# yhw-yhw/TalkSHOW

Hardware: AMD Instinct MI355X
Metric: generated SMPL-X frames/sec (10 s @ 30 fps clips), whole job (higher is better)
Workload: dtype f32; 1 GPU; BASELINE configs[1]: batch=32 x 10 s clips, body+hand VQ-VAE encode -> PixelCNN greedy decode -> VQ decode, 30 fps; batch_per_gpu=32, frames_per_clip=300, coalesce=8, streams=3

## Files before the change

include/talkshow_hip_debug.h:

```cpp
#ifndef TALKSHOW_HIP_DEBUG_H
#define TALKSHOW_HIP_DEBUG_H

#include "talkshow_hip.h"

#ifdef __cplusplus
extern "C" {
#endif

int ts_stream_create_cus(ts_ctx *ctx, int cu_first, int cu_count, void **out_stream);
int ts_debug_skinny_trace(unsigned long long *out, int max_records);
int ts_debug_clock_sample(unsigned long long *dev_out, int n, int window_us, void *stream);
int ts_debug_conv_bands(int M, int N, int groups, int *out4);
int ts_debug_split_tile(int bid, int MT, int NT, int gw, int *out2);
int ts_debug_tile_weights(const float *W, int N, int K, long ldw, int epi, int gateD, float *out);

int ts_op_conv1d_timed(ts_ctx *ctx, const float *x_dev, int B, int Lin, int Cin, const float *w_packed_dev,
                       const float *bias_dev, int Cout, int K, int tile, int iters, float *out_dev, float *ms_out,
                       void *stream);
int ts_op_conv1d_strided_timed(ts_ctx *ctx, const float *x_dev, int B, int Lin, int Cin, const float *w_packed_dev,
                               const float *bias_dev, int Cout, int K, int stride, int tile, int iters, float *out_dev,
                               float *ms_out, void *stream);

int ts_op_conv_taps48_timed(ts_ctx *ctx, const float *x_dev, int B, int T, int G, int ntap, const float *w_dev, const float *bias_dev,
                            const float *res_dev, int iters, float *out_dev, float *ms_out, void *stream);
// ... 102 lines not shown
int ts_debug_mfcc_mel(ts_mfcc *m, const float *power, const int32_t *frames_dev, int B, int T, float *mel, void *stream);
int ts_debug_mfcc_db(ts_mfcc *m, float *mel, const int32_t *frames_dev, int B, int T, void *stream);
int ts_debug_mfcc_dct(ts_mfcc *m, const float *mel, const int32_t *frames_dev, int B, int T, float *feat, void *stream);

int ts_debug_smplx_dims(const ts_smplx *m, int32_t *out5);
int ts_debug_smplx_need(const ts_smplx *m, int32_t *verts_out);
int ts_debug_smplx_pose_prepare(ts_smplx *m, const float *betas, int betas_per_row, const float *rows, int row_ld, int expr_off, int64_t N,
                                float *rot_out, float *X_out, void *stream);
int ts_debug_smplx_blend(ts_smplx *m, int which, const float *X, int64_t N, float *out, void *stream);
int ts_debug_smplx_rigid_chain(ts_smplx *m, const float *rot, const float *jrest, int64_t N, float *G_out, float *A_out, float *joints_out,
                               void *stream);
int ts_debug_smplx_skin(ts_smplx *m, int full, const float *vposed, const float *A, int64_t N, float *out, void *stream);
int ts_debug_smplx_joints_tail(ts_smplx *m, const float *vs, int64_t N, float *joints, void *stream);

int ts_debug_pixelcnn_graphs(ts_pixelcnn *pix, void *stream);

int ts_debug_code_tables_plan(int V, int D, int B, int r, int j, int last_row, const char *knob_list, int64_t *out12);
int ts_debug_pixelcnn_tables(ts_pixelcnn *pix, int mode);
int64_t ts_debug_pixelcnn_work(ts_pixelcnn *pix, void *stream, int which, float *buf_dev, int64_t cap_floats, int put);
int ts_debug_code_table_stage(ts_pixelcnn *pix, int which, const int32_t *tok_dev, int B, const float *add1, const float *add2, const float *cls,
                              float *pre, float *out, float *q1, float *q0, void *stream);

int ts_debug_mixed_plan(const int32_t *hrows, int B, int max_counts, int32_t *active_out);

int ts_debug_rep_table(const ts_repeat *rep_host, int n_rep, int B, int V, int32_t *words_out);

int ts_op_vq_argmin_pair_masked(ts_ctx *ctx, const float *z_body_dev, const float *z_hand_dev, const int32_t *lens_dev, int B, int H_max,
                                const float *codebook_body_dev, const float *codebook_hand_dev, int ncode_body, int ncode_hand, int dim_body,
                                int dim_hand, int64_t *codes_dev, void *stream);
int ts_debug_vq_argmin_pair_masked(ts_ctx *ctx, const float *z_body_dev, const float *z_hand_dev, const int32_t *lens_dev, int B, int H_max,
                                   const float *codebook_body_dev, const float *codebook_hand_dev, int ncode_body, int ncode_hand,
                                   int dim_body, int dim_hand, int64_t *codes_dev, int form, int iters, void *stream);

int ts_debug_skinny_chain(ts_ctx *ctx, int M, int K, int gate, int iters, int debug, float *us_out);

#ifdef __cplusplus
}
#endif
#endif
```

talkshow_amd/_lib.py:

```python
import ctypes as C
import os

import numpy as np
import torch

_HERE = os.path.dirname(os.path.abspath(__file__))
LIB_PATH = os.environ.get("TS_LIB_PATH") or os.path.join(_HERE, "lib", "libtalkshow_hip.so")

TS_SAMPLE_GREEDY, TS_SAMPLE_UNIFORMS, TS_SAMPLE_PHILOX, TS_TEACHER_FORCED = 0, 1, 2, 3


class TsTensor(C.Structure):
    _fields_ = [("name", C.c_char_p), ("data", C.POINTER(C.c_float)), ("ndim", C.c_int32), ("shape", C.c_int64 * 4)]


_vp, _i, _i64, _u64, _fp = C.c_void_p, C.c_int, C.c_int64, C.c_uint64, C.POINTER(C.c_float)


class TsSampling(C.Structure):
    _fields_ = [("temperature", C.c_float), ("top_p", C.c_float), ("top_k", C.c_int32), ("reserved", C.c_int32)]


_sp = C.POINTER(TsSampling)

# ... 113 lines not shown
    "ts_resample_kaiser": (_i, [_vp, _vp, _i, C.c_long, _i, _i, _vp, _vp]),
    "ts_mfcc_forward_mixed": (_i, [_vp, _vp, C.POINTER(C.c_int32), _vp, _i, C.c_long, _vp, _vp]),
    "ts_mfcc_resample_mixed": (_i, [_vp, _vp, C.POINTER(C.c_int32), _vp, _i, C.c_long, _vp, _vp]),
    "ts_resample_kaiser_mixed": (_i, [_vp, _vp, C.POINTER(C.c_int32), _vp, _i, C.c_long, _i, _i, _vp, _vp]),
    "ts_debug_mfcc_stft": (_i, [_vp, _vp, _i, C.c_long, _vp, _vp]),
    "ts_debug_mfcc_stft_lens": (_i, [_vp, _vp, C.POINTER(C.c_int32), _vp, _i, C.c_long, _vp, _vp]),
    "ts_debug_mfcc_frames": (_i, [_vp, _vp, _i, C.c_long, _vp, _vp]),
    "ts_debug_mfcc_mel": (_i, [_vp, _vp, _vp, _i, _i, _vp, _vp]),
    "ts_debug_mfcc_db": (_i, [_vp, _vp, _vp, _i, _i, _vp]),
    "ts_debug_mfcc_dct": (_i, [_vp, _vp, _vp, _i, _i, _vp, _vp]),
    "ts_pixelcnn_graph_stats": (_i, [_vp, _vp, _i, _i, _i, C.POINTER(_i64), C.POINTER(C.c_double)]),
    "ts_body_pixel_infer": (_i, [_vp, _vp, _vp, _vp, _vp, _vp, _i, _i, _i, _vp, _u64, _i64, _vp, _vp, _vp]),
    "ts_body_pixel_infer_mixed": (_i, [_vp, _vp, _vp, _vp, _vp, _vp, C.POINTER(C.c_int32), _vp, _i, _i, _i, _vp, _u64, _vp, _vp, _vp, _vp]),
    "ts_audioenc_forward_masked": (_i, [_vp, _vp, _vp, _i, _i, _vp, _vp]),
    "ts_pixelcnn_generate_mixed": (_i, [_vp, _vp, _vp, C.POINTER(C.c_int32), _vp, _i, _i, _i, _vp, _u64, _vp, _vp, _vp]),
    "ts_vqvae_decode_pair_masked": (_i, [_vp, _vp, _vp, _vp, _vp, _i, _i, _vp, _vp]),
    "ts_debug_mixed_plan": (_i, [C.POINTER(C.c_int32), _i, _i, C.POINTER(C.c_int32)]),
    "ts_body_vq_infer": (_i, [_vp, _vp, _vp, _i, _i, _vp, _vp, _vp]),
    "ts_op_conv1d": (_i, [_vp, _vp, _i, _i, _i, _fp, _fp, _i, _i, _i, _i, _i, _i, _vp, _vp]),
    "ts_op_conv1d_timed": (_i, [_vp, _vp, _i, _i, _i, _vp, _vp, _i, _i, _i, _i, _vp, C.POINTER(C.c_float), _vp]),
    "ts_op_conv_taps48_timed": (_i, [_vp, _vp, _i, _i, _i, _i, _vp, _vp, _vp, _i, _vp, C.POINTER(C.c_float), _vp]),
    "ts_op_conv1d_strided_timed": (_i, [_vp, _vp, _i, _i, _i, _vp, _vp, _i, _i, _i, _i, _i, _vp, C.POINTER(C.c_float), _vp]),
    "ts_debug_pixelcnn_graphs": (_i, [_vp, _vp]),
    "ts_debug_code_tables_plan": (_i, [_i, _i, _i, _i, _i, _i, C.c_char_p, C.POINTER(_i64)]),
    "ts_debug_pixelcnn_tables": (_i, [_vp, _i]),
    "ts_debug_pixelcnn_work": (_i64, [_vp, _vp, _i, _vp, _i64, _i]),
    "ts_debug_code_table_stage": (_i, [_vp, _i, _vp, _i, _vp, _vp, _vp, _vp, _vp, _vp, _vp, _vp]),
    "ts_debug_conv_run": (_i, [_vp, C.POINTER(ConvProblem), _i, C.c_char_p, _i, C.POINTER(_i), _vp]),
    "ts_debug_conv_sk_plan": (_i, [_i, _i, _i, _i, C.POINTER(C.c_int)]),
    "ts_debug_conv_sk_run": (_i, [_i, _i, _i, _i, C.POINTER(C.c_int)]),
    "ts_debug_conv_sk_supported": (_i, []),
    "ts_pixelcnn_graph_captures": (C.c_long, [_vp, _vp]),
    "ts_pixelcnn_prepare": (_i, [_vp, _i, _i, _i, _vp]),
    "ts_debug_conv_plan": (_i, [_i, _i, _i, _i, _i, C.POINTER(_i), _i, _i, C.c_char_p, C.POINTER(_i)]),
    "ts_debug_skinny_plan": (_i, [C.POINTER(_i), _i, C.c_char_p, C.POINTER(_i)]),
    "ts_debug_skinny_run": (_i, [_vp, C.POINTER(SkinnyProblem), _i, C.c_char_p, C.POINTER(_i), _vp]),
    "ts_debug_gate_act": (_i, [_vp, _vp, _vp, C.c_long, _vp]),
    "ts_debug_gelu": (_i, [_vp, _vp, C.c_long, _vp]),
    "ts_debug_attention": (_i, [_vp, _i, _i, _i, _i, C.c_float, _vp, _vp]),
    "ts_debug_layernorm_rows": (_i, [_vp, _i, C.c_long, _i, _vp, _vp, _vp, _i, _i, _vp, _i, _vp]),
    "ts_debug_lerp_ln": (_i, [_vp, _i, _i, _i, _vp, _vp, _vp, _vp]),
    "ts_debug_w2v_conv0": (_i, [_vp, _i, _i, _vp, _vp, _vp, _i, _vp, _vp]),
    "ts_debug_fill_id": (_i, [_vp, _i, _vp, _vp, _i, _vp, _i, _i, _i, _i, _vp]),
    "ts_debug_attention_mixed": (_i, [_vp, C.POINTER(C.c_int32), _vp, _i, _i, _i, _i, C.c_float, _vp, _vp]),
    "ts_debug_layernorm_rows_lens": (_i, [_vp, _i, _i, _i, _vp, _i, _vp, _vp, _vp, _i, _i, _vp, _i, _vp]),
    "ts_debug_lerp_ln_lens": (_i, [_vp, _i, _i, _i, _vp, _vp, _vp, _vp, _vp, _vp]),
    "ts_debug_w2v_conv0_lens": (_i, [_vp, _i, _i, _vp, _vp, _vp, _vp, _i, _vp, _vp]),
    "ts_debug_fill_id_lens": (_i, [_vp, _i, _vp, _vp, _i, _vp, _i, _i, _i, _i, _vp, _vp]),
    "ts_debug_face_mixed_grid": (_i, [C.POINTER(C.c_int32), _i, _i, C.POINTER(C.c_int32), _i]),
    "ts_debug_face_packed_layout": (_i, [C.POINTER(C.c_int32), C.POINTER(C.c_int32), _i, C.POINTER(_i64), C.POINTER(_i64), C.POINTER(_i64)]),
    "ts_debug_face_generate_mixed": (_i, [_vp, _vp, C.POINTER(C.c_int32), _vp, C.POINTER(C.c_int32), _vp, _i, _i, _i, _vp, _vp, _vp, _vp, _i]),
    "ts_debug_attention_packed": (_i, [_vp, C.POINTER(C.c_int32), _vp, _i, _i, _i, C.c_float, _vp, _vp]),
    "ts_debug_pack_rows": (_i, [_vp, C.POINTER(C.c_int32), _i, _i, _i, _vp, _vp]),
    "ts_debug_unpack_rows": (_i, [_vp, C.POINTER(C.c_int32), _vp, _i, _i, _i, _vp, _vp]),
    "ts_debug_w2v_conv0_packed": (_i, [_vp, _i, _i, C.POINTER(C.c_int32), _vp, _vp, _vp, _vp, _i, _vp, _vp]),
    "ts_debug_lerp_ln_packed": (_i, [_vp, _i, _i, C.POINTER(C.c_int32), _vp, _vp, _vp, _vp, _vp, _vp]),
    "ts_op_vq_argmin": (_i, [_vp, _vp, _i, _vp, _i, _i, _vp, _vp]),
    "ts_op_linear": (_i, [_vp, _vp, _i, _i, _fp, _fp, _i, _i, _vp, _vp]),
    "ts_op_sample": (_i, [_vp, _vp, _i, _i, _i, _vp, _vp, _vp]),
    "ts_op_sample_philox": (_i, [_vp, _vp, _i, _i, _u64, _i64, C.c_uint32, _vp, _vp]),
    "ts_debug_skinny_chain": (_i, [_vp, _i, _i, _i, _i, _i, C.POINTER(C.c_float)]),
    "ts_smplx_create": (_i, [_vp, _i, _i, _i, _i, _fp, _fp, _fp, _fp, C.POINTER(C.c_int32), _fp, _fp, C.POINTER(C.c_int32), _i,
                             C.POINTER(C.c_int32), _i, C.POINTER(C.c_int32), _fp, _i, C.POINTER(_vp)]),
    "ts_smplx_destroy": (None, [_vp]),
    "ts_smplx_num_joints": (_i, [_vp]),
    "ts_smplx_forward": (_i, [_vp, _vp, _i, _vp, _i, _i, _i64, _vp, _vp, _vp]),
# ... 595 lines not shown
```

talkshow_amd/csrc/api.cpp:

```cpp
#include <cstring>
#include <vector>
#include "host_common.h"
#include "conv_tile.h"
#include "skinny_desc.h"

using namespace ts;

namespace {
struct BodyWork {
    DevBuf feat;
    DevBuf lat[2];
    DevBuf given;
};
BodyWork &body_work(hipStream_t s) {
    static StreamWorks<BodyWork> works;
    return works.get(s);
}
}

namespace ts {
template <class Get>
static Knobs read_knobs(Get get) {
    Knobs v;
    auto num = [&](const char *name, int dflt) { const char *e = get(name); return e && e[0] ? std::atoi(e) : dflt; };
    v.conv_bands = num("TS_CONV_BANDS", 1) != 0;
    v.conv_ring = num("TS_CONV_RING", 9);
    v.conv_deal = num("TS_CONV_DEAL", 1) != 0;
    v.conv_ring_paired = num("TS_CONV_RING_PAIRED", 1) != 0;
    v.conv_taps48 = num("TS_CONV_TAPS48", 1) != 0;
    v.face_pack = num("TS_FACE_PACK", 0) != 0;
    v.conv_sk = num("TS_CONV_SK", 1);
    v.w2v_moments = num("TS_W2V_MOMENTS", 1) != 0;
    v.vq_lds = num("TS_VQ_LDS", 1) != 0;
    v.vq_pair = num("TS_VQ_PAIR", 1) != 0;
    v.split_xcd = num("TS_SPLIT_XCD", 8);
    v.prof_log = num("TS_PROF_LOG", 0) != 0;
    if (const char *e = get("TS_NO_GRAPH")) v.no_graph = e[0] && e[0] != '0';
    v.pix_defer_p = num("TS_PIX_DEFER_P", -1);
    v.pix_tables = num("TS_PIX_TABLES", -1);
    v.skinny_v = num("TS_SKINNY_V", 1);
    v.skinny_nt = num("TS_SKINNY_NT", 16);
    v.skinny_tiled = num("TS_SKINNY_TILED", 1) != 0;
    v.wide_min = num("TS_SKINNY_WIDE_MIN", 160);
    v.skinny_shape = num("TS_SKINNY_SHAPE", 0);
    v.skinny_trace = num("TS_SKINNY_TRACE", 0);
    v.wide_ablate = num("TS_SKINNY_WIDE_ABLATE", 0);
    v.wide_pair = num("TS_SKINNY_WIDE_PAIR", 1) != 0;
    return v;
}
const Knobs &knobs() {
    static const Knobs k = read_knobs([](const char *name) { return std::getenv(name); });
    return k;
}
static Knobs knobs_from_list(const char *list) {
    return read_knobs([list](const char *name) -> const char * {
        const size_t n = std::strlen(name);
        for (const char *q = list; q && (q = std::strstr(q, name)); q += n)
            if ((q == list || q[-1] == ',' || q[-1] == ' ') && q[n] == '=') return q + n + 1;
        return nullptr;
    });
}
}

extern "C" {
// ... 1114 lines not shown
    sp.tok32 = tok.i();
    sp.tok_stride = 1;
    sp.codes = idx;
    sp.code_stride = 1;
    TS_HIP(launch_sample(sp, s));
    TS_HIP(hipStreamSynchronize(s));
    return 0;
}

int ts_op_sample_philox(ts_ctx *ctx, const float *logits, int B, int V, uint64_t seed, int64_t clip_index0, uint32_t position,
                        int64_t *idx, void *stream) {
    if (!ctx || !logits || !idx) return fail("ts_op_sample_philox: null argument");
    hipStream_t s = (hipStream_t)stream;
    DevBuf tok;
    TS_TRY(tok.ensure((size_t)B * sizeof(int)));
    SampleParams sp;
    std::memset(&sp, 0, sizeof(sp));
    sp.logits = logits;
    sp.B = B;
    sp.V = V;
    sp.mode = TS_SAMPLE_PHILOX;
    sp.seed = seed;
    sp.clip_index0 = clip_index0;
    sp.position = position;
    sp.tok32 = tok.i();
    sp.tok_stride = 1;
    sp.codes = idx;
    sp.code_stride = 1;
    TS_HIP(launch_sample(sp, s));
    TS_HIP(hipStreamSynchronize(s));
    return 0;
}

}
```

talkshow_amd/csrc/host_common.h:

```cpp
#pragma once
#include <hip/hip_runtime.h>

#include <cmath>
#include <cstring>
#include <map>
#include <atomic>
#include <memory>
#include <mutex>
#include <string>
#include <vector>

#include "../../include/talkshow_hip.h"
#include "../../include/talkshow_hip_debug.h"
#include "kernels.h"

namespace ts {

void set_error(const std::string &m);
inline int fail(const std::string &m) {
    set_error(m);
    return 1;
}

#define TS_HIP(expr)                                                                              \
// ... 137 lines not shown
    ts::Profiler prof;
    std::atomic<long> n_launch[ts::FAM_COUNT] = {};
    std::atomic<double> n_flops[ts::FAM_COUNT] = {};
    ts::DevBuf neg1;
};

namespace ts {

int run_conv(ts_ctx *ctx, const ConvParams &p, int tile, hipStream_t s);
int run_skinny(ts_ctx *ctx, const SkinnyParams &p, hipStream_t s);
int run_skinny_batch(ts_ctx *ctx, const SkinnyParams *const *ps, int n, hipStream_t s);
struct MiscScope {
    ts_ctx *ctx;
    hipStream_t s;
    MiscScope(ts_ctx *c, hipStream_t st, int fam = FAM_MISC, double flops = 0.0) : ctx(c), s(st) {
        if (ctx->prof.on) {
            ctx->prof.begin(fam, s);
            ctx->prof.flops[fam] += flops;
        }
    }
    ~MiscScope() {
        if (ctx->prof.on) ctx->prof.end(s);
    }
};

struct ConvLayer {
    int kind = 0;
    int cin = 0, cin_pad = 0, cout = 0, cout_pad = 0, npad = 0, ktot = 0;
    int act = 0;
    int ngroups = 1, nseg = 0;
    ConvSeg segs[2][4];
    DevBuf w, bias;
    DevBuf wp;
    std::string name;
};

int pack_conv_layer(const StateDict &sd, const std::string &conv_key, const std::string &norm_key,
                    const std::string &res_key, int kind, int k, int cin, int cout, int act, ConvLayer *out);
int pack_linear_layer(const float *w, long ldw, const float *bias, int N, int K, ConvLayer *out);

int pack_conv_raw(const float *w, const float *bias, int cout, int cin, int K, const int *taps, int act, ConvLayer *out);

int conv_layer_params(const ConvLayer &layer, const float *x, int ldx, int B, int Lin, const float *res, int ldr,
                      float *out, int ldo, int out_col0, int n_store, ConvParams *p);

int convnet_hidden(const ts_convnet *n);
int face_mixed_grid(const int32_t *frames, int B, int heads, std::vector<int> &work);
struct FacePacked {
    std::vector<int> feat_off, row0;
    long feat_rows = 0, rows = 0;
    int len[7] = {};
};
constexpr int FACE_FC_K[6] = {3, 3, 3, 3, 2, 2};
int face_packed_layout(const int32_t *ns, const int32_t *frames, int B, FacePacked *out);
int vqvae_in_dim(const ts_vqvae *v);
int vq_encode_pair_masked(ts_vqvae *vb, ts_vqvae *vh, const float *poses, int poses_ld, const int32_t *lens_dev, int B, int T_max, int64_t *codes,
                          int codes_H, float *z_body, float *z_hand, int form, hipStream_t s);

struct MixedPass {
    const int64_t *ids;
    const int32_t *lens_host, *lens_dev;
    int B, rows, mode;
    const float *uniforms;
    uint64_t seed;
    const int64_t *clip_index;
    int64_t *codes;
};
struct MixedOpts {
    const ts_sampling *ctl_host = nullptr;
    int n_ctl = 0;
    float *logprob = nullptr;
    const int64_t *given = nullptr;
    const int32_t *given_rows_host = nullptr;
    const uint8_t *keep = nullptr;
    const float *style = nullptr;
    int style_rows = 0;
    const float *bias = nullptr;
// ... 22 lines not shown
```

talkshow_amd/csrc/kernels.h:

```cpp
#pragma once
#include <hip/hip_runtime.h>
#include <stdint.h>

namespace ts {

struct Knobs;

struct ConvSeg {
    int d;
    int c0;
    int len;
    int ntap;
};

struct ConvGroup {
    const float *x;
    const float *w;
    const float *bias;
    const float *res;
    float *out;
    int out_col0;
    int nseg;
    ConvSeg seg[4];
};
// ... 61 lines not shown
bool conv_taps48_takes(const ConvParams &p);

enum class ConvEngine { Reg, RegBanded, Ring, RingDealt, RingBanded, RingSK, Taps48, Split, Invalid };
struct ConvPlan {
    ConvEngine engine = ConvEngine::Invalid;
    int bm = 0, bn = 0, wm = 0, wn = 0, bk = 32;
    int planes = 0;
    ConvBands bands{};
    ConvSK sk{};
};
ConvPlan plan_conv(const ConvParams &p, int tile, const Knobs &k, bool sk_hw);
const char *conv_plan_refusal(const ConvParams &p, const ConvPlan &plan);
hipError_t launch_conv_plan(const ConvParams &p, const ConvPlan &plan, hipStream_t stream);
hipError_t launch_conv_gemm(const ConvParams &p, int tile, hipStream_t stream);

__host__ __device__ inline bool split_tile_of(int bid, int MT, int NT, int GW, int &tx, int &ty) {
    const int total = MT * NT, per = (total + 7) >> 3;
    const int L = (bid & 7) * per + (bid >> 3);
    if (L >= total) return false;
    const int full = NT / GW;
    int g = L / (MT * GW), r = L - g * MT * GW, gn = GW;
    if (g >= full) {
        g = full;
        r = L - full * MT * GW;
        gn = NT - GW * full;
    }
    tx = r / gn;
    ty = g * GW + (r - tx * gn);
    return true;
}

hipError_t launch_split_weight_planes(const float *w, float *planes, long rows, int K, hipStream_t stream);
double conv_gemm_flops(const ConvParams &p);

struct SkinnySeg {
    const float *base;
    const int *gidx;
    long row_stride;
    long gidx_stride;
    int row_shift;
    int len;
    int tiled_w;
};

enum { EPI_LINEAR = 0, EPI_GATE = 1 };
constexpr int SKINNY_MAX_SEG = 3;
constexpr int SKINNY_MAX_PROBLEMS = 6;

struct SkinnyParams {
    int M, N;
    int nseg, Ktot;
    SkinnySeg seg[SKINNY_MAX_SEG];
    const float *W;
    long ldw;
    const float *bias;
    const float *add1;
    long add1_stride;
    int add1_shift;
    const float *add2;
    long add2_stride;
    int add2_shift;
    const float *add3;
    long add3_stride;
    const float *clsrow;
    int cls_ld;
    int epi;
// ... 102 lines not shown
                                float *out, hipStream_t stream);
hipError_t launch_assemble_full_lens(const float *body, const int *tb, const float *face, const int *tf, const float *lower_pose33, int B,
                                     int Tb, int Tf, float *out, hipStream_t stream);
hipError_t launch_i64_to_i32(const int64_t *src, int *dst, long n, hipStream_t stream);
hipError_t launch_gate_act(const float *v, const float *p, float *out, long n, hipStream_t stream);
hipError_t launch_gelu(const float *v, float *out, long n, hipStream_t stream);
hipError_t launch_set_words3(uint64_t *dst, uint64_t a, uint64_t b, uint64_t c, hipStream_t stream);
hipError_t launch_clock_sample(unsigned long long *out, int n, unsigned long long window_ticks, hipStream_t stream);

struct Knobs {
    bool conv_bands = true;
    bool vq_lds = true;
    bool vq_pair = true;
    int conv_ring = 9;
    bool w2v_moments = true;
    int conv_sk = 1;
    bool face_pack = false;
    bool conv_taps48 = true;
    bool conv_ring_paired = true;
    bool conv_deal = true;
    int split_xcd = 8;
    bool prof_log = false;
    bool no_graph = false;
    int pix_defer_p = -1;
    int pix_tables = -1;
    int skinny_v = 1;
    int skinny_nt = 16;
    bool skinny_tiled = true;
    int wide_min = 160;
    int skinny_shape = 0;
    int skinny_trace = 0;
    bool wide_pair = true;
    int wide_ablate = 0;
};
const Knobs &knobs();

constexpr size_t CODE_TABLE_CAP_BYTES = (size_t)192 << 20;
constexpr int CODE_TABLE_MIN_CLIPS = 64;
struct CodeTablePlan {
    bool fits = false;
    int waves_v0 = 0, sets_v0 = 0, waves_hg = 0;
    size_t bytes_v0 = 0, bytes_hg = 0;
};
inline CodeTablePlan code_table_plan(int V, int D, const Knobs &k) {
    CodeTablePlan t;
    if (V < 1 || D < 32 || D % 32) return t;
    t.waves_v0 = code_table_waves(2 * D);
    t.sets_v0 = 1 + t.waves_v0 / 2;
    t.waves_hg = code_table_waves(D);
    t.bytes_v0 = (size_t)3 * t.sets_v0 * V * 4 * D * sizeof(float);
    t.bytes_hg = (size_t)V * 2 * D * sizeof(float);
    t.fits = k.skinny_nt != 32 && (size_t)V * 4 * D * sizeof(float) * 15 <= CODE_TABLE_CAP_BYTES;
    return t;
}
inline bool code_table_pass(bool built, int mode, int B) { return built && (mode > 0 || (mode < 0 && B >= CODE_TABLE_MIN_CLIPS)); }
inline bool code_table_v0_row(int r) { return r >= 1; }
inline bool code_table_hg_col(int j) { return j == 1; }
inline bool code_table_rider(int r, int t, int last_row) { return r >= 1 && r + (2 - t) < last_row; }


__device__ __forceinline__ float erf_fast(float x) {
    const float a = __builtin_fabsf(x), t = a * a;
    float p = __builtin_fmaf(t, -0.000561801774892956f, 0.004913816228508949f);
    p = __builtin_fmaf(t, p, -0.026707515120506287f);
    p = __builtin_fmaf(t, p, 0.11280010640621185f);
    p = __builtin_fmaf(t, p, -0.37612295150756836f);
// ... 146 lines not shown
```

talkshow_amd/csrc/models.cpp:

```cpp
#include <cstdio>
#include "host_common.h"

namespace ts {

static thread_local std::string g_err;
void set_error(const std::string &m) { g_err = m; }
const char *last_error() { return g_err.c_str(); }

namespace {
std::mutex &scoped_mu() {
    static std::mutex m;
    return m;
}
std::vector<StreamScoped *> &scoped_all() {
    static std::vector<StreamScoped *> v;
    return v;
}
}
StreamScoped::StreamScoped() {
    std::lock_guard<std::mutex> g(scoped_mu());
    scoped_all().push_back(this);
}
StreamScoped::~StreamScoped() {
    std::lock_guard<std::mutex> g(scoped_mu());
    auto &v = scoped_all();
    for (size_t i = 0; i < v.size(); ++i)
        if (v[i] == this) {
            v[i] = v.back();
            v.pop_back();
            break;
        }
}
void drop_stream_everywhere(hipStream_t s) {
    std::lock_guard<std::mutex> g(scoped_mu());
// ... 150 lines not shown
    L->cout_pad = round_up(cout, 32);
    L->npad = round_up(cout, 128);
    L->act = act;
    L->name = conv_key;
    const int cp = L->cin_pad;
    std::vector<std::pair<int, int>> taps[2];
    if (kind == 0) {
        L->ngroups = 1;
        if (K == 1) taps[0] = {{0, 0}};
        else if (K == 3) taps[0] = {{-1, 0}, {0, 1}, {1, 2}};
        else return fail("pack_conv_layer: unsupported kernel size");
    } else if (kind == 1) {
        L->ngroups = 1;
        taps[0] = {{-1, 0}, {0, 1}, {1, 2}, {2, 3}};
    } else {
        L->ngroups = 2;
        taps[0] = {{-1, 3}, {0, 1}};
        taps[1] = {{0, 2}, {1, 0}};
    }
    L->nseg = (int)taps[0].size();
    L->ktot = L->nseg * cp;
    std::vector<float> wp((size_t)L->ngroups * L->npad * L->ktot, 0.f), bp((size_t)L->ngroups * L->npad, 0.f);
    for (int g = 0; g < L->ngroups; ++g) {
        for (int s = 0; s < L->nseg; ++s) {
            L->segs[g][s] = ConvSeg{taps[g][s].first, 0, cp};
            for (int o = 0; o < cout; ++o)
                for (int i = 0; i < cin; ++i)
                    wp[((size_t)g * L->npad + o) * L->ktot + (size_t)s * cp + i] = W(o, i, taps[g][s].second);
        }
        for (int o = 0; o < cout; ++o) bp[(size_t)g * L->npad + o] = c[o] + (br ? br[o] : 0.f);
    }
    TS_TRY(L->w.upload(wp.data(), wp.size() * sizeof(float)));
    TS_TRY(L->bias.upload(bp.data(), bp.size() * sizeof(float)));
    return 0;
}

int pack_conv_raw(const float *w, const float *bias, int cout, int cin, int K, const int *taps, int act, ConvLayer *L) {
    if (K > 4) return fail("pack_conv_raw: at most 4 taps");
    L->kind = 0;
    L->cin = cin;
    L->cin_pad = round_up(cin, 32);
    L->cout = cout;
    L->cout_pad = round_up(cout, 32);
    L->npad = round_up(cout, 128);
    L->act = act;
    L->ngroups = 1;
    L->nseg = K;
    const int cp = L->cin_pad;
    L->ktot = K * cp;
    std::vector<float> wp((size_t)L->npad * L->ktot, 0.f), bp(L->npad, 0.f);
    for (int s = 0; s < K; ++s) {
        L->segs[0][s] = ConvSeg{taps[s], 0, cp, 1};
        for (int o = 0; o < cout; ++o)
            for (int i = 0; i < cin; ++i) wp[(size_t)o * L->ktot + (size_t)s * cp + i] = w[((size_t)o * cin + i) * K + s];
    }
    if (bias)
        for (int o = 0; o < cout; ++o) bp[o] = bias[o];
    TS_TRY(L->w.upload(wp.data(), wp.size() * sizeof(float)));
    TS_TRY(L->bias.upload(bp.data(), bp.size() * sizeof(float)));
    return 0;
}

int pack_linear_layer(const float *w, long ldw, const float *bias, int N, int K, ConvLayer *L) {
    L->kind = 0;
    L->cin = K;
    L->cin_pad = round_up(K, 32);
    L->cout = N;
    L->cout_pad = round_up(N, 32);
    L->npad = round_up(N, 128);
    L->act = 0;
    L->ngroups = 1;
    L->nseg = 1;
    L->ktot = L->cin_pad;
    L->segs[0][0] = ConvSeg{0, 0, L->cin_pad};
    std::vector<float> wp((size_t)L->npad * L->ktot, 0.f), bp(L->npad, 0.f);
    for (int o = 0; o < N; ++o) {
        for (int i = 0; i < K; ++i) wp[(size_t)o * L->ktot + i] = w[(long)o * ldw + i];
        if (bias) bp[o] = bias[o];
    }
    TS_TRY(L->w.upload(wp.data(), wp.size() * sizeof(float)));
    TS_TRY(L->bias.upload(bp.data(), bp.size() * sizeof(float)));
    return 0;
}

int conv_layer_params(const ConvLayer &L, const float *x, int ldx, int B, int Lin, const float *res, int ldr,
                      float *out, int ldo, int out_col0, int n_store, ConvParams *p) {
    std::memset(p, 0, sizeof(*p));
    const int Lrows = L.kind == 1 ? Lin / 2 : Lin;
    p->M = B * Lrows;
    p->Lout = Lrows;
    p->Lin = Lin;
    p->stride = L.kind == 1 ? 2 : 1;
    p->ldx = ldx;
    p->ldr = ldr;
    p->N = n_store;
    p->Ktot = L.ktot;
    p->act = L.act;
    p->ngroups = L.ngroups;
    for (int g = 0; g < L.ngroups; ++g) {
        ConvGroup &G = p->g[g];
        G.x = x;
        G.w = L.w.f() + (size_t)g * L.npad * L.ktot;
        G.bias = L.bias.f() + (size_t)g * L.npad;
        G.res = res;
        G.out = out;
        G.nseg = L.nseg;
        for (int s = 0; s < L.nseg; ++s) G.seg[s] = L.segs[g][s];
        if (L.kind == 2) {
            G.out_col0 = g * ldo + out_col0;
        } else {
            G.out_col0 = out_col0;
        }
    }
    p->ldo = L.kind == 2 ? 2 * ldo : ldo;
    return L.kind == 2 ? 2 * Lin : Lrows;
}

}

using namespace ts;

namespace {

struct Stack {
    std::vector<std::unique_ptr<ConvLayer>> layers;
    ConvLayer tail;
};

int pack_stack(const StateDict &sd, const std::string &p, int c, int nres, Stack *st) {
    for (int i = 0; i < nres; ++i) {
        st->layers.emplace_back(new ConvLayer());
        const std::string q = p + "._layers." + std::to_string(i);
        TS_TRY(pack_conv_layer(sd, q + ".conv", q + ".norm", "", 0, 3, c, c, 1, st->layers.back().get()));
    }
    TS_TRY(pack_conv_layer(sd, p + ".conv", p + ".norm", "", 0, 3, c, c, 2, &st->tail));
    return 0;
}

struct Pool {
    DevBuf slab;
    size_t each = 0;
    int live[2] = {-1, -1};
    int ensure(size_t floats_each) {
        each = (floats_each + 63) / 64 * 64;
        return slab.ensure(4 * each * sizeof(float));
    }
    float *buf(int i) const { return slab.f() + (size_t)i * each; }
    int pick(int a, int b = -1, int c = -1) const {
        for (int i = 0; i < 4; ++i)
            if (i != a && i != b && i != c) return i;
        return 0;
    }
};

}

struct ts_convnet {
    ts_ctx *ctx = nullptr;
    int in_dim = 0, hid = 0, nres = 0;
    ConvLayer project, down1, down2;
    Stack s1, s2, s3;
    bool has_pre_vq = false;
    ConvLayer pre_vq;
    struct Work {
        Pool pool;
        DevBuf xin;
    };
    StreamWorks<Work> works;
    Work &work(hipStream_t s) { return works.get(s); }
};

namespace {

int pack_trunk(ts_ctx *ctx, const StateDict &sd, const std::string &p, int in_dim, int hid, int nres, ts_convnet *n) {
    if (hid % 128 != 0) return fail("num_hiddens must be a multiple of 128 (channel tiles are 32 wide)");
    n->ctx = ctx;
    n->in_dim = in_dim;
    n->hid = hid;
    n->nres = nres;
    TS_TRY(pack_conv_layer(sd, p + "project.conv", p + "project.norm", "", 0, 3, in_dim, hid / 4, 1, &n->project));
// ... 12 lines not shown
    int shr, shl;
};

int run_layer_n(ts_ctx *ctx, int n, const ConvLayer *const *L, const float *const *x, int ldx, int B, int Lin,
                const float *const *res, int ldr, float *const *out, int ldo, const int *col0, const int *nstore,
                hipStream_t s, int *Lout, const LenMask *mk = nullptr) {
    ConvParams p[2];
    for (int i = 0; i < n; ++i) {
        *Lout = conv_layer_params(*L[i], x[i], ldx, B, Lin, res ? res[i] : nullptr, ldr, out[i], ldo, col0 ? col0[i] : 0,
                                  nstore[i], &p[i]);
        if (mk) p[i].lens = mk->lens, p[i].len_shr = mk->shr, p[i].len_shl = mk->shl;
    }
    bool same = n == 2 && L[0]->kind == L[1]->kind && L[0]->cin_pad == L[1]->cin_pad && L[0]->ktot == L[1]->ktot &&
                L[0]->act == L[1]->act && L[0]->ngroups == L[1]->ngroups && nstore[0] == nstore[1] &&
                2 * L[0]->ngroups <= 4;
    if (same) {
        ConvParams &q = p[0];
        for (int g = 0; g < L[1]->ngroups; ++g) q.g[q.ngroups + g] = p[1].g[g];
        q.ngroups += L[1]->ngroups;
        return run_conv(ctx, q, 0, s);
    }
    for (int i = 0; i < n; ++i) TS_TRY(run_conv(ctx, p[i], 0, s));
    return 0;
}

int run_layer(ts_ctx *ctx, const ConvLayer &L, const float *x, int ldx, int B, int Lin, const float *res, int ldr,
              float *out, int ldo, int col0, int nstore, hipStream_t s, int *Lout, const LenMask *mk = nullptr) {
    const ConvLayer *Lp[1] = {&L};
    const float *xp[1] = {x}, *rp[1] = {res};
    float *op[1] = {out};
    return run_layer_n(ctx, 1, Lp, xp, ldx, B, Lin, rp, ldr, op, ldo, &col0, &nstore, s, Lout, mk);
}

int run_stack_n(ts_ctx *ctx, int n, const Stack *const *st, Pool *const *pool, int cur, int c, int B, int L, hipStream_t s,
                int *out_idx, const LenMask *mk = nullptr) {
    int h = cur, tmp = 0;
    const int ns[2] = {c, c};
    const ConvLayer *Lp[2];
    const float *xp[2], *rp[2];
    float *op[2];
    for (size_t k = 0; k < st[0]->layers.size(); ++k) {
        const int o = pool[0]->pick(cur, h);
        for (int i = 0; i < n; ++i) { Lp[i] = st[i]->layers[k].get(); xp[i] = pool[i]->buf(h); op[i] = pool[i]->buf(o); }
        TS_TRY(run_layer_n(ctx, n, Lp, xp, c, B, L, nullptr, 0, op, c, nullptr, ns, s, &tmp, mk));
        h = o;
    }
    const int o = pool[0]->pick(cur, h);
    for (int i = 0; i < n; ++i) { Lp[i] = &st[i]->tail; xp[i] = pool[i]->buf(h); rp[i] = pool[i]->buf(cur); op[i] = pool[i]->buf(o); }
    TS_TRY(run_layer_n(ctx, n, Lp, xp, c, B, L, rp, c, op, c, nullptr, ns, s, &tmp, mk));
    *out_idx = o;
    return 0;
}

int run_trunk_n(int n, ts_convnet *const *net, const float *const *x, int x_ld, int B, int T, hipStream_t s, int *out_idx,
                int *H, const int *lens = nullptr) {
    if (T < 4) return fail("sequence too short: need T >= 4 frames");
    LenMask m0{lens, 0, 0}, m1{lens, 1, 0}, m2{lens, 2, 0};
    const LenMask *k0 = lens ? &m0 : nullptr, *k1 = lens ? &m1 : nullptr, *k2 = lens ? &m2 : nullptr;
    ts_ctx *ctx = net[0]->ctx;
    const int hid = net[0]->hid;
    Pool *pool[2];
    const float *xin[2];
    int ldx[2];
    for (int i = 0; i < n; ++i) {
        if (net[i]->hid != hid) return fail("paired networks must have the same width");
        ts_convnet::Work &wk = net[i]->work(s);
        pool[i] = &wk.pool;
        TS_TRY(pool[i]->ensure((size_t)B * T * (hid / 4)));
        xin[i] = x[i];
        ldx[i] = net[i]->in_dim;
        if (net[i]->in_dim % 32 != 0 || lens) {
            const int cp = net[i]->project.cin_pad;
            TS_TRY(wk.xin.ensure((size_t)B * T * cp * sizeof(float)));
            MiscScope ms(ctx, s);
            const int xl = x_ld > 0 ? x_ld : net[i]->in_dim;
            if (lens) TS_HIP(launch_pad_rows_masked(x[i], xl, net[i]->in_dim, wk.xin.f(), cp, cp, B, T, lens, s));
            else TS_HIP(launch_pad_rows(x[i], xl, net[i]->in_dim, wk.xin.f(), cp, cp, (long)B * T, s));
            xin[i] = wk.xin.f();
            ldx[i] = cp;
        } else if (x_ld > 0) {
            ldx[i] = x_ld;
        }
    }
    int L = T, tmp = 0, cur = 0, o = 0;
    const ConvLayer *Lp[2];
    const Stack *Sp[2];
    const float *xp[2];
    float *op[2];
    int ns[2];
    for (int i = 0; i < n; ++i)
        TS_TRY(run_layer(ctx, net[i]->project, xin[i], ldx[i], B, L, nullptr, 0, pool[i]->buf(0), hid / 4, 0, hid / 4, s, &tmp, k0));
    for (int i = 0; i < n; ++i) Sp[i] = &net[i]->s1;
    TS_TRY(run_stack_n(ctx, n, Sp, pool, cur, hid / 4, B, L, s, &o, k0));
    cur = o;
    o = pool[0]->pick(cur);
    for (int i = 0; i < n; ++i) { Lp[i] = &net[i]->down1; xp[i] = pool[i]->buf(cur); op[i] = pool[i]->buf(o); ns[i] = hid / 2; }
    TS_TRY(run_layer_n(ctx, n, Lp, xp, hid / 4, B, L, nullptr, 0, op, hid / 2, nullptr, ns, s, &L, k1));
    cur = o;
    for (int i = 0; i < n; ++i) Sp[i] = &net[i]->s2;
    TS_TRY(run_stack_n(ctx, n, Sp, pool, cur, hid / 2, B, L, s, &o, k1));
    cur = o;
// ... 61 lines not shown
        for (int i = 0; i < n; ++i) {
            if (vq[i]->ncode == 0) continue;
            TS_HIP(launch_vq_argmin(zp[i], vq[i]->emb, B * H, vq[i]->codebook.f(), vq[i]->code_sq.f(), vq[i]->ncode, vq[i]->emb,
                                    lat_out[i], 1, s));
            if (q_out && q_out[i])
                TS_HIP(launch_gather_rows(vq[i]->codebook.f(), vq[i]->emb, vq[i]->ncode, lat_out[i], 1, B * H, vq[i]->emb, q_out[i], vq[i]->emb, s));
        }
    }
    *Hout = H;
    return 0;
}

int vq_encode_impl(ts_vqvae *vq, const float *poses, int poses_ld, int B, int T, float *z_out, int64_t *lat_out,
                   float *q_out, hipStream_t s, int *Hout) {
    ts_vqvae *vp[1] = {vq};
    const float *pp[1] = {poses};
    float *zp[1] = {z_out}, *qp[1] = {q_out};
    int64_t *lp[1] = {lat_out};
    return vq_encode_n(1, vp, pp, poses_ld, B, T, zp, lp, qp, s, Hout);
}

int vq_decode_n(int n, ts_vqvae *const *vq, const int64_t *const *lat, const float *const *z, int B, int H, float *out,
                int out_ld, const int *col0, hipStream_t s, const int *lens = nullptr) {
    ts_ctx *ctx = vq[0]->ctx;
    LenMask m0{lens, 2, 0}, m1{lens, 2, 1}, m2{lens, 2, 2};
    const LenMask *k0 = lens ? &m0 : nullptr, *k1 = lens ? &m1 : nullptr, *k2 = lens ? &m2 : nullptr;
    if (lens && z) return fail("length-masked decode takes code indices");
    const int hid = vq[0]->hid;
    Pool *pool[2];
    for (int i = 0; i < n; ++i) {
        if (vq[i]->hid != hid) return fail("paired VQ-VAEs must have the same width");
        pool[i] = &vq[i]->work(s).pool;
        TS_TRY(pool[i]->ensure((size_t)B * H * hid));
        if (z && z[i]) {
            int tmp = 0;
            TS_TRY(run_layer(ctx, vq[i]->aft, z[i], vq[i]->emb, B, H, nullptr, 0, pool[i]->buf(0), hid, 0, hid, s, &tmp));
        } else {
            if (vq[i]->ncode == 0) return fail("this network has no codebook (auto-encoder): decode continuous latents");
            MiscScope ms(ctx, s);
            if (lens) TS_HIP(launch_gather_rows_masked(vq[i]->aft_table.f(), hid, vq[i]->ncode, lat[i], 1, B * H, hid, pool[i]->buf(0), hid, H, lens, 2, s));
            else TS_HIP(launch_gather_rows(vq[i]->aft_table.f(), hid, vq[i]->ncode, lat[i], 1, B * H, hid, pool[i]->buf(0), hid, s));
        }
    }
    int cur = 0, o = 0, L = H;
    const ConvLayer *Lp[2];
    const Stack *Sp[2];
    const float *xp[2];
    float *op[2];
    int ns[2];
    for (int i = 0; i < n; ++i) Sp[i] = &vq[i]->d1;
    TS_TRY(run_stack_n(ctx, n, Sp, pool, cur, hid, B, L, s, &o, k0));
    cur = o;
    o = pool[0]->pick(cur);
    for (int i = 0; i < n; ++i) { Lp[i] = &vq[i]->up2; xp[i] = pool[i]->buf(cur); op[i] = pool[i]->buf(o); ns[i] = hid / 2; }
    TS_TRY(run_layer_n(ctx, n, Lp, xp, hid, B, L, nullptr, 0, op, hid / 2, nullptr, ns, s, &L, k0));
    cur = o;
    for (int i = 0; i < n; ++i) Sp[i] = &vq[i]->d2;
    TS_TRY(run_stack_n(ctx, n, Sp, pool, cur, hid / 2, B, L, s, &o, k1));
    cur = o;
    o = pool[0]->pick(cur);
    for (int i = 0; i < n; ++i) { Lp[i] = &vq[i]->up3; xp[i] = pool[i]->buf(cur); op[i] = pool[i]->buf(o); ns[i] = hid / 4; }
    TS_TRY(run_layer_n(ctx, n, Lp, xp, hid / 2, B, L, nullptr, 0, op, hid / 4, nullptr, ns, s, &L, k1));
    cur = o;
    for (int i = 0; i < n; ++i) Sp[i] = &vq[i]->d3;
    TS_TRY(run_stack_n(ctx, n, Sp, pool, cur, hid / 4, B, L, s, &o, k2));
    int tmp = 0;
// ... 303 lines not shown
```

Before: 1.737 million frames/s.

## Lower stride-1 k=3 residual conv stacks to Winograd F(4,3) batched GEMMs

```diff
diff --git a/include/talkshow_hip_debug.h b/include/talkshow_hip_debug.h
--- a/include/talkshow_hip_debug.h
+++ b/include/talkshow_hip_debug.h
@@ -158,6 +158,13 @@
                                    const float *codebook_body_dev, const float *codebook_hand_dev, int ncode_body, int ncode_hand,
                                    int dim_body, int dim_hand, int64_t *codes_dev, int form, int iters, void *stream);
 
+int ts_debug_wino_lowering(int cin, int cout, int k, int stride, const char *knob_list, int B, int L, int *out5);
+int ts_debug_wino_weights(const float *w, int cout, int cin, float *out);
+int ts_debug_wino_transform(ts_ctx *ctx, int which, int nnet, int B, int L, int C, int act, const int32_t *lens_dev, int shr, int shl,
+                            const void *const *ptrs, void *stream);
+int ts_debug_wino_gemm(ts_ctx *ctx, int nnet, const float *V0, const float *V1, const float *U0, const float *U1, float *O0, float *O1, int M,
+                       int C, void *stream);
+
 int ts_debug_skinny_chain(ts_ctx *ctx, int M, int K, int gate, int iters, int debug, float *us_out);
 
 #ifdef __cplusplus
diff --git a/talkshow_amd/_lib.py b/talkshow_amd/_lib.py
--- a/talkshow_amd/_lib.py
+++ b/talkshow_amd/_lib.py
@@ -169,6 +169,10 @@
     "ts_debug_conv_sk_supported": (_i, []),
     "ts_pixelcnn_graph_captures": (C.c_long, [_vp, _vp]),
     "ts_pixelcnn_prepare": (_i, [_vp, _i, _i, _i, _vp]),
+    "ts_debug_wino_lowering": (_i, [_i, _i, _i, _i, C.c_char_p, _i, _i, C.POINTER(_i)]),
+    "ts_debug_wino_weights": (_i, [_vp, _i, _i, _vp]),
+    "ts_debug_wino_transform": (_i, [_vp, _i, _i, _i, _i, _i, _i, _vp, _i, _i, C.POINTER(_vp), _vp]),
+    "ts_debug_wino_gemm": (_i, [_vp, _i, _vp, _vp, _vp, _vp, _vp, _vp, _i, _i, _vp]),
     "ts_debug_conv_plan": (_i, [_i, _i, _i, _i, _i, C.POINTER(_i), _i, _i, C.c_char_p, C.POINTER(_i)]),
     "ts_debug_skinny_plan": (_i, [C.POINTER(_i), _i, C.c_char_p, C.POINTER(_i)]),
     "ts_debug_skinny_run": (_i, [_vp, C.POINTER(SkinnyProblem), _i, C.c_char_p, C.POINTER(_i), _vp]),
diff --git a/talkshow_amd/csrc/api.cpp b/talkshow_amd/csrc/api.cpp
--- a/talkshow_amd/csrc/api.cpp
+++ b/talkshow_amd/csrc/api.cpp
@@ -30,6 +30,7 @@
     v.conv_taps48 = num("TS_CONV_TAPS48", 1) != 0;
     v.face_pack = num("TS_FACE_PACK", 0) != 0;
     v.conv_sk = num("TS_CONV_SK", 1);
+    v.conv_wino = num("TS_CONV_WINO", -1);
     v.w2v_moments = num("TS_W2V_MOMENTS", 1) != 0;
     v.vq_lds = num("TS_VQ_LDS", 1) != 0;
     v.vq_pair = num("TS_VQ_PAIR", 1) != 0;
@@ -1210,4 +1211,46 @@
     return 0;
 }
 
-}
+int ts_debug_wino_lowering(int cin, int cout, int k, int stride, const char *knob_list, int B, int L, int *out5) {
+    if (cin < 1 || cout < 1 || k < 1 || stride < 1 || B < 1 || L < 1 || !out5) return -1;
+    const ts::Knobs kn = ts::knobs_from_list(knob_list);
+    if (stride != 1 || !ts::wino_lowered(0, k, cin, cout, kn.conv_wino)) return 0;
+    const int o[5] = {6, B * ((L + 3) / 4), cout, cin, 4};
+    std::memcpy(out5, o, sizeof(o));
+    return 1;
+}
+
+int ts_debug_wino_weights(const float *w, int cout, int cin, float *out) {
+    if (!w || !out || cout < 1 || cin < 1) return fail("ts_debug_wino_weights: bad argument");
+    ts::wino_transform_weights(w, cout, cin, round_up(cout, 128), out);
+    return 0;
+}
+
+int ts_debug_wino_transform(ts_ctx *ctx, int which, int nnet, int B, int L, int C, int act, const int32_t *lens_dev, int shr, int shl,
+                            const void *const *ptrs, void *stream) {
+    if (!ctx || !ptrs || nnet < 1 || nnet > 2) return fail("ts_debug_wino_transform: bad argument");
+    ts::WinoParams w;
+    std::memset(&w, 0, sizeof(w));
+    w.nnet = nnet;
+    w.B = B, w.L = L, w.J = (L + 3) / 4, w.C = C, w.act = act;
+    w.lens = lens_dev, w.len_shr = shr, w.len_shl = shl;
+    for (int i = 0; i < nnet; ++i) {
+        const void *const *q = ptrs + 6 * i;
+        w.x[i] = (const float *)q[0], w.V[i] = (float *)q[1], w.O[i] = (const float *)q[2], w.bias[i] = (const float *)q[3];
+        w.res[i] = (const float *)q[4], w.y[i] = (float *)q[5];
+    }
+    MiscScope ms(ctx, (hipStream_t)stream);
+    TS_HIP(ts::launch_wino(which, w, (hipStream_t)stream));
+    return 0;
+}
+
+int ts_debug_wino_gemm(ts_ctx *ctx, int nnet, const float *V0, const float *V1, const float *U0, const float *U1, float *O0, float *O1, int M,
+                       int C, void *stream) {
+    if (!ctx || nnet < 1 || nnet > 2 || !V0 || !U0 || !O0 || (nnet == 2 && (!V1 || !U1 || !O1)) || M < 1 || C < 32 || C % 32)
+        return fail("ts_debug_wino_gemm: bad argument");
+    const float *V[2] = {V0, V1}, *U[2] = {U0, U1};
+    float *O[2] = {O0, O1};
+    return ts::run_wino_gemm(ctx, nnet, V, U, O, M, C, round_up(C, 128), (hipStream_t)stream);
+}
+
+}
diff --git a/talkshow_amd/csrc/conv_wino.hip b/talkshow_amd/csrc/conv_wino.hip
--- /dev/null
+++ b/talkshow_amd/csrc/conv_wino.hip
@@ -0,0 +1,170 @@
+#include "kernels.h"
+#include "conv_tile.h"
+
+namespace ts {
+
+namespace {
+
+__device__ __forceinline__ f32x4 ld4(const float *p) { return *reinterpret_cast<const f32x4 *>(p); }
+__device__ __forceinline__ void st4(float *p, f32x4 v) { *reinterpret_cast<f32x4 *>(p) = v; }
+
+__device__ __forceinline__ void wino_bt(const f32x4 (&d)[6], f32x4 (&v)[6]) {
+#pragma clang fp contract(off)
+    v[0] = (4.f * d[0] - 5.f * d[2]) + d[4];
+    v[1] = ((d[3] - 4.f * d[1]) - 4.f * d[2]) + d[4];
+    v[2] = ((4.f * d[1] - 4.f * d[2]) - d[3]) + d[4];
+    v[3] = ((2.f * d[3] - 2.f * d[1]) - d[2]) + d[4];
+    v[4] = ((2.f * d[1] - d[2]) - 2.f * d[3]) + d[4];
+    v[5] = (4.f * d[1] - 5.f * d[3]) + d[5];
+}
+
+__device__ __forceinline__ f32x4 wino_at_row(const f32x4 (&m)[6], const int r) {
+#pragma clang fp contract(off)
+    if (r == 0) return (((m[0] + m[1]) + m[2]) + m[3]) + m[4];
+    if (r == 1) return ((m[1] - m[2]) + 2.f * m[3]) - 2.f * m[4];
+    if (r == 2) return ((m[1] + m[2]) + 4.f * m[3]) + 4.f * m[4];
+    return (((m[1] - m[2]) + 8.f * m[3]) - 8.f * m[4]) + m[5];
+}
+
+__device__ __forceinline__ f32x4 wino_finish(f32x4 y, const f32x4 bias, const float *res, const int act) {
+#pragma clang fp contract(off)
+    f32x4 v = y + bias;
+    if (res) v = v + ld4(res);
+#pragma unroll
+    for (int q = 0; q < 4; ++q) {
+        float e = v[q];
+        if (act == 1) e = e >= 0.f ? e : e * 0.2f;
+        else if (act == 2) e = e > 0.f ? e : 0.f;
+        else if (act == 3) e = gelu_fast(e);
+        v[q] = e;
+    }
+    return v;
+}
+
+struct WinoItem {
+    int net, b, j, c, Lb;
+    long row;
+    bool ok;
+};
+__device__ __forceinline__ WinoItem wino_item(const WinoParams &p) {
+    WinoItem w;
+    const int c4 = p.C >> 2;
+    const long idx = (long)blockIdx.x * blockDim.x + threadIdx.x;
+    w.net = blockIdx.y;
+    w.row = idx / c4;
+    w.c = (int)(idx - w.row * c4) << 2;
+    w.ok = w.row < (long)p.B * p.J;
+    w.b = (int)(w.row / p.J);
+    w.j = (int)(w.row - (long)w.b * p.J);
+    w.Lb = p.L;
+    if (w.ok && p.lens) {
+        const int l = (p.lens[w.b] >> p.len_shr) << p.len_shl;
+        w.Lb = l < p.L ? l : p.L;
+    }
+    return w;
+}
+
+__device__ __forceinline__ void wino_load_tile(const float *O, const long comp_stride, const long row, const int C, const int c, f32x4 (&m)[6]) {
+#pragma unroll
+    for (int i = 0; i < 6; ++i) m[i] = ld4(O + i * comp_stride + row * C + c);
+}
+
+__global__ __launch_bounds__(256) void wino_in_kernel(const WinoParams p) {
+    const WinoItem w = wino_item(p);
+    if (!w.ok) return;
+    const float *x = p.x[w.net] + (long)w.b * p.L * p.C + w.c;
+    f32x4 d[6], v[6];
+#pragma unroll
+    for (int k = 0; k < 6; ++k) {
+        const int t = 4 * w.j - 1 + k;
+        d[k] = t >= 0 && t < w.Lb ? ld4(x + (long)t * p.C) : f32x4{0.f, 0.f, 0.f, 0.f};
+    }
+    wino_bt(d, v);
+    const long cs = (long)p.B * p.J * p.C;
+    float *V = p.V[w.net] + w.row * p.C + w.c;
+#pragma unroll
+    for (int i = 0; i < 6; ++i) st4(V + i * cs, v[i]);
+}
+
+__global__ __launch_bounds__(256) void wino_out_kernel(const WinoParams p) {
+    const WinoItem w = wino_item(p);
+    if (!w.ok) return;
+    const long cs = (long)p.B * p.J * p.C;
+    f32x4 m[6];
+    wino_load_tile(p.O[w.net], cs, w.row, p.C, w.c, m);
+    const f32x4 bias = ld4(p.bias[w.net] + w.c);
+    const float *res = p.res[w.net];
+    float *y = p.y[w.net] + (long)w.b * p.L * p.C + w.c;
+#pragma unroll
+    for (int r = 0; r < 4; ++r) {
+        const int t = 4 * w.j + r;
+        if (t >= p.L) break;
+        f32x4 v{0.f, 0.f, 0.f, 0.f};
+        if (t < w.Lb) v = wino_finish(wino_at_row(m, r), bias, res ? res + ((long)w.b * p.L + t) * p.C + w.c : nullptr, p.act);
+        st4(y + (long)t * p.C, v);
+    }
+}
+
+__global__ __launch_bounds__(256) void wino_out_in_kernel(const WinoParams p) {
+    const WinoItem w = wino_item(p);
+    if (!w.ok) return;
+    const long cs = (long)p.B * p.J * p.C;
+    const float *O = p.O[w.net];
+    const f32x4 bias = ld4(p.bias[w.net] + w.c);
+    const f32x4 zero{0.f, 0.f, 0.f, 0.f};
+    f32x4 m[6], d[6], v[6];
+    d[0] = zero;
+    if (w.j > 0 && 4 * w.j - 1 < w.Lb) {
+        wino_load_tile(O, cs, w.row - 1, p.C, w.c, m);
+        d[0] = wino_finish(wino_at_row(m, 3), bias, nullptr, p.act);
+    }
+    wino_load_tile(O, cs, w.row, p.C, w.c, m);
+#pragma unroll
+    for (int r = 0; r < 4; ++r) d[1 + r] = 4 * w.j + r < w.Lb ? wino_finish(wino_at_row(m, r), bias, nullptr, p.act) : zero;
+    d[5] = zero;
+    if (w.j + 1 < p.J && 4 * w.j + 4 < w.Lb) {
+        wino_load_tile(O, cs, w.row + 1, p.C, w.c, m);
+        d[5] = wino_finish(wino_at_row(m, 0), bias, nullptr, p.act);
+    }
+    wino_bt(d, v);
+    float *V = p.V[w.net] + w.row * p.C + w.c;
+#pragma unroll
+    for (int i = 0; i < 6; ++i) st4(V + i * cs, v[i]);
+}
+
+}
+
+hipError_t launch_wino(int which, const WinoParams &p, hipStream_t stream) {
+    if (p.nnet < 1 || p.nnet > 2 || p.B < 1 || p.L < 1 || p.C < 4 || (p.C & 3) || p.J != (p.L + 3) / 4 || p.act < 0 || p.act > 3 ||
+        (p.lens && (p.len_shr < 0 || p.len_shl < 0)))
+        return hipErrorInvalidValue;
+    const long items = (long)p.B * p.J * (p.C >> 2);
+    if (items + 255 >= (1l << 31)) return hipErrorInvalidValue;
+    for (int n = 0; n < p.nnet; ++n) {
+        const bool in = which == 0 ? p.x[n] && p.V[n] : which == 1 ? p.O[n] && p.bias[n] && p.y[n] : p.O[n] && p.bias[n] && p.V[n];
+        if (!in) return hipErrorInvalidValue;
+    }
+    const dim3 grid((unsigned)((items + 255) / 256), p.nnet);
+    if (which == 0) hipLaunchKernelGGL(wino_in_kernel, grid, dim3(256), 0, stream, p);
+    else if (which == 1) hipLaunchKernelGGL(wino_out_kernel, grid, dim3(256), 0, stream, p);
+    else if (which == 2) hipLaunchKernelGGL(wino_out_in_kernel, grid, dim3(256), 0, stream, p);
+    else return hipErrorInvalidValue;
+    return hipGetLastError();
+}
+
+void wino_transform_weights(const float *w, int cout, int cin, int npad, float *out) {
+    static const double G[6][3] = {{1.0 / 4, 0, 0},          {-1.0 / 6, -1.0 / 6, -1.0 / 6}, {-1.0 / 6, 1.0 / 6, -1.0 / 6},
+                                   {1.0 / 24, 1.0 / 12, 1.0 / 6}, {1.0 / 24, -1.0 / 12, 1.0 / 6}, {0, 0, 1}};
+    for (int i = 0; i < 6; ++i)
+        for (int o = 0; o < npad; ++o)
+            for (int c = 0; c < cin; ++c) {
+                double u = 0.0;
+                if (o < cout) {
+                    const float *g = w + ((size_t)o * cin + c) * 3;
+                    u = G[i][0] * (double)g[0] + G[i][1] * (double)g[1] + G[i][2] * (double)g[2];
+                }
+                out[((size_t)i * npad + o) * cin + c] = (float)u;
+            }
+}
+
+}
diff --git a/talkshow_amd/csrc/host_common.h b/talkshow_amd/csrc/host_common.h
--- a/talkshow_amd/csrc/host_common.h
+++ b/talkshow_amd/csrc/host_common.h
@@ -193,6 +193,7 @@
     ConvSeg segs[2][4];
     DevBuf w, bias;
     DevBuf wp;
+    DevBuf wino;
     std::string name;
 };
 
@@ -204,6 +205,8 @@
 
 int conv_layer_params(const ConvLayer &layer, const float *x, int ldx, int B, int Lin, const float *res, int ldr,
                       float *out, int ldo, int out_col0, int n_store, ConvParams *p);
+
+int run_wino_gemm(ts_ctx *ctx, int n, const float *const *V, const float *const *U, float *const *O, int M, int c, int npad, hipStream_t s);
 
 int convnet_hidden(const ts_convnet *n);
 int face_mixed_grid(const int32_t *frames, int B, int heads, std::vector<int> &work);
diff --git a/talkshow_amd/csrc/kernels.h b/talkshow_amd/csrc/kernels.h
--- a/talkshow_amd/csrc/kernels.h
+++ b/talkshow_amd/csrc/kernels.h
@@ -117,6 +117,27 @@
 
 hipError_t launch_split_weight_planes(const float *w, float *planes, long rows, int K, hipStream_t stream);
 double conv_gemm_flops(const ConvParams &p);
+
+constexpr int WINO_MIN_C = 512;
+inline bool wino_lowered(int kind, int k, int cin, int cout, int knob) {
+    const bool geom = kind == 0 && k == 3 && cin == cout && cin % 32 == 0;
+    return geom && knob != 0 && (knob == 1 || cout >= WINO_MIN_C);
+}
+struct WinoParams {
+    int nnet;
+    int B, L, J, C;
+    int act;
+    const int *lens;
+    int len_shr, len_shl;
+    const float *x[2];
+    float *V[2];
+    const float *O[2];
+    const float *bias[2];
+    const float *res[2];
+    float *y[2];
+};
+hipError_t launch_wino(int which, const WinoParams &p, hipStream_t stream);
+void wino_transform_weights(const float *w, int cout, int cin, int npad, float *out);
 
 struct SkinnySeg {
     const float *base;
@@ -285,6 +306,7 @@
     int skinny_trace = 0;
     bool wide_pair = true;
     int wide_ablate = 0;
+    int conv_wino = -1;
 };
 const Knobs &knobs();
 
diff --git a/talkshow_amd/csrc/models.cpp b/talkshow_amd/csrc/models.cpp
--- a/talkshow_amd/csrc/models.cpp
+++ b/talkshow_amd/csrc/models.cpp
@@ -1,5 +1,7 @@
+#include <algorithm>
 #include <cstdio>
 #include "host_common.h"
+#include "conv_tile.h"
 
 namespace ts {
 
@@ -216,6 +218,14 @@
     }
     TS_TRY(L->w.upload(wp.data(), wp.size() * sizeof(float)));
     TS_TRY(L->bias.upload(bp.data(), bp.size() * sizeof(float)));
+    if (wino_lowered(kind, K, cin, cout, knobs().conv_wino)) {
+        std::vector<float> w3((size_t)cout * cin * 3), u((size_t)6 * L->npad * cin);
+        for (int o = 0; o < cout; ++o)
+            for (int i = 0; i < cin; ++i)
+                for (int kk = 0; kk < 3; ++kk) w3[((size_t)o * cin + i) * 3 + kk] = W(o, i, kk);
+        wino_transform_weights(w3.data(), cout, cin, L->npad, u.data());
+        TS_TRY(L->wino.upload(u.data(), u.size() * sizeof(float)));
+    }
     return 0;
 }
 
@@ -265,6 +275,35 @@
     TS_TRY(L->w.upload(wp.data(), wp.size() * sizeof(float)));
     TS_TRY(L->bias.upload(bp.data(), bp.size() * sizeof(float)));
     return 0;
+}
+
+int run_wino_gemm(ts_ctx *ctx, int n, const float *const *V, const float *const *U, float *const *O, int M, int c, int npad, hipStream_t s) {
+    auto dist = [](const float *a, const float *b) { return (long)((reinterpret_cast<intptr_t>(a) - reinterpret_cast<intptr_t>(b)) / (intptr_t)sizeof(float)); };
+    ConvParams p;
+    std::memset(&p, 0, sizeof(p));
+    p.M = p.Lout = p.Lin = M;
+    p.stride = 1;
+    p.ldx = p.ldo = c;
+    p.N = c;
+    p.Ktot = c;
+    p.ngroups = 6 * n;
+    p.zdiv = 6;
+    ConvGroup &g = p.g[0];
+    g.x = V[0];
+    g.w = U[0];
+    g.out = O[0];
+    g.nseg = 1;
+    g.seg[0] = ConvSeg{0, 0, c, 1};
+    p.x_zs1 = p.o_zs1 = (long)M * c;
+    p.w_zs1 = (long)npad * c;
+    if (n == 2) {
+        p.x_zs0 = dist(V[1], V[0]);
+        p.o_zs0 = dist(O[1], O[0]);
+        p.w_zs0 = dist(U[1], U[0]);
+    }
+    const ConvPlan pl = plan_conv(p, 0, knobs(), false);
+    const bool ring = pl.engine == ConvEngine::Reg && pl.bm == 128 && pl.bn == 128 && knobs().conv_ring > 0 && conv_gemm_ring_takes(p);
+    return run_conv(ctx, p, ring ? 35 : 0, s);
 }
 
 int conv_layer_params(const ConvLayer &L, const float *x, int ldx, int B, int Lin, const float *res, int ldr,
@@ -330,6 +369,12 @@
         return slab.ensure(4 * each * sizeof(float));
     }
     float *buf(int i) const { return slab.f() + (size_t)i * each; }
+    DevBuf wv, wo;
+    int ensure_wino(size_t floats) {
+        if (floats == 0) return 0;
+        TS_TRY(wv.ensure(floats * sizeof(float)));
+        return wo.ensure(floats * sizeof(float));
+    }
     int pick(int a, int b = -1, int c = -1) const {
         for (int i = 0; i < 4; ++i)
             if (i != a && i != b && i != c) return i;
@@ -408,8 +453,57 @@
     return run_layer_n(ctx, 1, Lp, xp, ldx, B, Lin, rp, ldr, op, ldo, &col0, &nstore, s, Lout, mk);
 }
 
+size_t stack_wino_floats(const Stack &st, int c, int B, int L) {
+    return st.tail.wino.p ? (size_t)6 * round_up(B * ((L + 3) / 4), 128) * c : 0;
+}
+
+int run_stack_wino(ts_ctx *ctx, int n, const Stack *const *st, Pool *const *pool, int cur, int c, int B, int L, hipStream_t s, int *out_idx,
+                   const LenMask *mk) {
+    WinoParams w;
+    std::memset(&w, 0, sizeof(w));
+    w.nnet = n;
+    w.B = B, w.L = L, w.J = (L + 3) / 4, w.C = c;
+    if (mk) w.lens = mk->lens, w.len_shr = mk->shr, w.len_shl = mk->shl;
+    const int o = pool[0]->pick(cur), M = B * w.J;
+    for (int i = 0; i < n; ++i) {
+        if (pool[i]->wv.bytes < (size_t)6 * M * c * sizeof(float) || pool[i]->wo.bytes < (size_t)6 * M * c * sizeof(float))
+            return fail("run_stack_wino: the Winograd arenas were not grown for this pass");
+        w.x[i] = pool[i]->buf(cur);
+        w.V[i] = pool[i]->wv.f();
+        w.O[i] = pool[i]->wo.f();
+        w.res[i] = pool[i]->buf(cur);
+        w.y[i] = pool[i]->buf(o);
+    }
+    const ConvLayer *Lp[2];
+    {
+        MiscScope ms(ctx, s);
+        TS_HIP(launch_wino(0, w, s));
+    }
+    const size_t nl = st[0]->layers.size();
+    for (size_t k = 0; k <= nl; ++k) {
+        for (int i = 0; i < n; ++i) {
+            Lp[i] = k < nl ? st[i]->layers[k].get() : &st[i]->tail;
+            w.bias[i] = Lp[i]->bias.f();
+        }
+        w.act = Lp[0]->act;
+        const float *Vp[2] = {w.V[0], w.V[1]}, *Up[2] = {Lp[0]->wino.f(), n == 2 ? Lp[1]->wino.f() : nullptr};
+        float *Op[2] = {pool[0]->wo.f(), n == 2 ? pool[1]->wo.f() : nullptr};
+        TS_TRY(run_wino_gemm(ctx, n, Vp, Up, Op, M, c, Lp[0]->npad, s));
+        MiscScope ms(ctx, s);
+        TS_HIP(launch_wino(k < nl ? 2 : 1, w, s));
+    }
+    *out_idx = o;
+    return 0;
+}
+
 int run_stack_n(ts_ctx *ctx, int n, const Stack *const *st, Pool *const *pool, int cur, int c, int B, int L, hipStream_t s,
                 int *out_idx, const LenMask *mk = nullptr) {
+    bool wino = true;
+    for (int i = 0; i < n; ++i) {
+        wino = wino && st[i]->tail.wino.p;
+        for (const auto &l : st[i]->layers) wino = wino && l->wino.p;
+    }
+    if (wino) return run_stack_wino(ctx, n, st, pool, cur, c, B, L, s, out_idx, mk);
     int h = cur, tmp = 0;
     const int ns[2] = {c, c};
     const ConvLayer *Lp[2];
@@ -443,6 +537,8 @@
         ts_convnet::Work &wk = net[i]->work(s);
         pool[i] = &wk.pool;
         TS_TRY(pool[i]->ensure((size_t)B * T * (hid / 4)));
+        TS_TRY(pool[i]->ensure_wino(std::max({stack_wino_floats(net[i]->s1, hid / 4, B, T), stack_wino_floats(net[i]->s2, hid / 2, B, T / 2),
+                                              stack_wino_floats(net[i]->s3, hid, B, T / 4)})));
         xin[i] = x[i];
         ldx[i] = net[i]->in_dim;
         if (net[i]->in_dim % 32 != 0 || lens) {
@@ -570,6 +666,8 @@
         if (vq[i]->hid != hid) return fail("paired VQ-VAEs must have the same width");
         pool[i] = &vq[i]->work(s).pool;
         TS_TRY(pool[i]->ensure((size_t)B * H * hid));
+        TS_TRY(pool[i]->ensure_wino(std::max({stack_wino_floats(vq[i]->d1, hid, B, H), stack_wino_floats(vq[i]->d2, hid / 2, B, 2 * H),
+                                              stack_wino_floats(vq[i]->d3, hid / 4, B, 4 * H)})));
         if (z && z[i]) {
             int tmp = 0;
             TS_TRY(run_layer(ctx, vq[i]->aft, z[i], vq[i]->emb, B, H, nullptr, 0, pool[i]->buf(0), hid, 0, hid, s, &tmp));
```

Measured after the change: 2.012 million frames/s (median of 6 runs). 15.9% higher.
